# RaphaelHaddad/Real-Time-Brain-Inspired-Video-Memory

Hardware: NVIDIA B200
Metric: queries_per_sec_top10_384d (higher is better)
Workload: dtype tf32

## Files before the change

real-time-brain-inspired-video-memory_b200/csrc/api.cu:

```cuda
#include "common.cuh"

#include <dlfcn.h>
#include <stdarg.h>
#include <stdlib.h>
#include <string.h>
#include <time.h>
#include <new>
#include <vector>

namespace vm {

static thread_local char g_err[512] = "";
void set_error(const char *fmt, ...)
{
    va_list ap;
    va_start(ap, fmt);
    vsnprintf(g_err, sizeof(g_err), fmt, ap);
    va_end(ap);
}

int k_convert_rows(const void *src, int src_dtype, void *dst, int dst_dtype, int64_t n, int dim, int ld, cudaStream_t st);
int k_row_inv_norms(const void *rows, int dtype, float *inv_norms, int64_t row0, int64_t n, int ld, int *extreme, cudaStream_t st,
                    const double *exact = nullptr);
int k_invalidate_rows(float *inv_norms, const int64_t *rows_dev, int64_t n, int64_t size, cudaStream_t st);
// ... 217 lines not shown
static int ws_prepare(vm_store *s)
{
    Workspace &w = s->ws;
    if (w.ready) return VM_OK;
    int lists = 2 * s->sm_count;
    w.lists_max = lists;
    int rc;
#define ENS(b, bytes) if ((rc = (b).ensure(bytes)) != VM_OK) return rc
    ENS(w.q_raw, (size_t)MAXQ * s->dim * 8);
    ENS(w.q_f32, (size_t)MAXQ * s->ld * 4);
    ENS(w.q_bf16, (size_t)2 * MAXQ * s->ld * 2);
    ENS(w.cand, (size_t)lists * MAXQ * (MAXK > SCAN_SLAB ? MAXK : SCAN_SLAB) * 8);
    ENS(w.merged, (size_t)MAXQ * MAXK * 8);
    ENS(w.o_idx, result_bytes(MAXQ, MAXK) + 64);
    ENS(w.flags, (size_t)(MAXQ + 2) * 4);
    ENS(w.seed, (size_t)(SEED_TAB_WORDS + 3 * MAXQ) * 4);
    ENS(w.ubuf, (size_t)MAXQ * SCAN_UNION_CAP * 8);
    ENS(w.done, 64);
    ENS(w.scnt, (size_t)256 * MAXQ * 4);
    ENS(w.sel_inc, (size_t)MAXQ * 4);
    VM_CUDA_CHECK(cudaMemset(w.done.p, 0, 64));
    ENS(w.col_thr, (size_t)MAXQ * 4);
    ENS(w.col_cnt, (size_t)MAXQ * 4);
    ENS(w.col_buf, (size_t)MAXQ * COLLECT_CAP * 8);
    ENS(w.xs, (size_t)XCTAS * MAXQ * MAXK * 8);
    ENS(w.xr, (size_t)XCTAS * MAXQ * MAXK * 4);
    ENS(w.xc, (size_t)XCTAS * MAXQ * 4);
    ENS(w.taken, (size_t)MAXQ * XCTAS * MAXK);
#undef ENS
    VM_CUDA_CHECK(cudaMallocHost((void **)&w.h_uncert, 64));
    VM_CUDA_CHECK(cudaMallocHost((void **)&w.h_pack, result_bytes(MAXQ, MAXK) + 64));
// ... 973 lines not shown
    }
    delete c;
    return VM_OK;
}
extern "C" int vm_comm_nranks(const vm_comm *c) { return c ? c->nranks : -1; }
extern "C" int vm_comm_rank(const vm_comm *c) { return c ? c->rank : -1; }

extern "C" int vm_synth_fill(int device, void *rows_dev, int dtype, uint64_t seed, int64_t row0, int64_t n, int dim,
                             uint64_t dup_period, void *stream)
{
    VM_REQUIRE(rows_dev, VM_ERR_BADARG, "rows is NULL");
    VM_REQUIRE(dtype == VM_F32 || dtype == VM_BF16, VM_ERR_BADARG, "dtype must be VM_F32 or VM_BF16");
    DeviceGuard g(device);
    return k_synth_fill(rows_dev, dtype, seed, row0, n, dim, ld_for_dim(dim), dup_period, (cudaStream_t)stream);
}
```

real-time-brain-inspired-video-memory_b200/csrc/common.cuh:

```cuda
#pragma once
#include <cuda_runtime.h>
#include <cuda_bf16.h>
#include <stdint.h>
#include <stdio.h>
#include <math.h>
#include <utility>
#include "../../include/vidmem.h"

namespace vm {

void set_error(const char *fmt, ...);
#define VM_CUDA_CHECK(expr)                                                                      \
    do {                                                                                         \
        cudaError_t _e = (expr);                                                                 \
        if (_e != cudaSuccess) {                                                                 \
            vm::set_error("%s failed: %s (%s:%d)", #expr, cudaGetErrorString(_e), __FILE__, __LINE__); \
            return VM_ERR_CUDA;                                                                  \
        }                                                                                        \
    } while (0)
#define VM_REQUIRE(cond, code, ...)          \
    do {                                     \
        if (!(cond)) {                       \
            vm::set_error(__VA_ARGS__);      \
            return (code);                   \
// ... 16 lines not shown
    cfg.numAttrs = pdl ? 1 : 0;
    return cudaLaunchKernelEx(&cfg, kernel, std::forward<Args>(args)...);
}

template <auto Kernel>
static inline cudaError_t max_smem_once(int bytes)
{
    static bool set[64] = {};
    int dev = 0;
    cudaError_t e = cudaGetDevice(&dev);
    if (e != cudaSuccess || set[dev & 63]) return e;
    e = cudaFuncSetAttribute(Kernel, cudaFuncAttributeMaxDynamicSharedMemorySize, bytes);
    if (e == cudaSuccess) set[dev & 63] = true;
    return e;
}

__host__ __device__ __forceinline__ uint32_t f32_ordered(float f)
{
#ifdef __CUDA_ARCH__
    uint32_t b = __float_as_uint(f);
#else
    uint32_t b;
    memcpy(&b, &f, 4);
#endif
    return (b & 0x80000000u) ? ~b : (b | 0x80000000u);
}
__host__ __device__ __forceinline__ float f32_from_ordered(uint32_t o)
{
    uint32_t b = (o & 0x80000000u) ? (o & 0x7FFFFFFFu) : ~o;
#ifdef __CUDA_ARCH__
// ... 222 lines not shown
```

real-time-brain-inspired-video-memory_b200/csrc/scan_tc.cu:

```cuda
#include "tc_common.cuh"

namespace vm {
using namespace tc;

static constexpr int TC_BLOCK_M = 128;
static constexpr int TC_STAGE_BYTES = TC_BLOCK_M * 128;
static constexpr int TC_ACC = 8;
static constexpr int TC_THREADS_SVC = 288;
static constexpr int TC_THREADS = 192;
static constexpr int TC_TMEM_COLS = 512;
static constexpr int TC_MAX_STAGES = 8;

struct CollectArgs {
    const float *thr;
    uint64_t *buf;
    int *cnt;
    int cap;
    const int *pending;
};

struct BandArgs {
    uint64_t *slab;
    int *scnt;
    uint64_t *ubuf;
    int *ucnt;
    int ucap;
    float band;
    int ksel;
    int use_seed;
};

struct TcLayout {
    int nq_pad, KB, stages, split;
    uint32_t off_b, off_a, off_tauf, off_lcnt, off_cmax, off_wmax, off_flags, off_bars, off_tmem, total;
};

static TcLayout make_layout(int dtype, int ld, int nq, int split = 0)
{
    TcLayout L{};
    const int es = dtype == VM_F32 ? 4 : 2;
    L.nq_pad = (nq + 15) & ~15;
    L.KB = (ld * es + 127) / 128;
    L.split = (split && dtype == VM_BF16) ? 1 : 0;
    uint32_t o = 0;
    L.off_b = o; o += (uint32_t)L.KB * L.nq_pad * 128 * (L.split ? 2 : 1);
    const uint32_t epi = (uint32_t)L.nq_pad * (4 + 4 + 4 + 16) + 64 + 8 * (2 * TC_MAX_STAGES + 1 + 2 * TC_ACC) + 16;
    int64_t room = 227 * 1024 - 2048 - (int64_t)o - epi;
    L.stages = (int)(room / TC_STAGE_BYTES);
    if (L.stages > TC_MAX_STAGES) L.stages = TC_MAX_STAGES;
    if (L.stages < 0) L.stages = 0;
    L.off_a = o; o += (uint32_t)L.stages * TC_STAGE_BYTES;
    L.off_tauf = o; o += (uint32_t)L.nq_pad * 4;
    L.off_lcnt = o; o += (uint32_t)L.nq_pad * 4;
    L.off_cmax = o; o += (uint32_t)L.nq_pad * 4;
    L.off_wmax = o; o += (uint32_t)L.nq_pad * 16;
    L.off_flags = o; o += 64;
    L.off_bars = o; o += 8 * (2 * TC_MAX_STAGES + 1 + 2 * TC_ACC);
    L.off_tmem = o; o += 16;
    L.total = o + 1024;
#ifdef VIDMEM_AB_SMEMPAD
    if (L.total < 220 * 1024) L.total = 220 * 1024;
#endif
    return L;
}

__device__ __forceinline__ uint32_t own_kth_score(const uint64_t *slab, int n, int k, int lane)
{
    constexpr int PER = SCAN_SLAB / 32;
    uint32_t vals[PER];
#pragma unroll
    for (int t = 0; t < PER; ++t) {
        const int i = lane + 32 * t;
        vals[t] = i < n ? (uint32_t)(__ldcg(slab + i) >> 32) : 0u;
// ... 3 lines not shown
    for (int bit = 31; bit >= 12; --bit) {
        const uint32_t hi = bit == 31 ? 0u : (0xFFFFFFFFu << (bit + 1));
        int cnt = 0;
#pragma unroll
        for (int t = 0; t < PER; ++t) cnt += ((vals[t] & hi) == prefix && ((vals[t] >> bit) & 1u)) ? 1 : 0;
        const int tot = __reduce_add_sync(0xffffffffu, cnt);
        if (tot >= need) prefix |= 1u << bit;
        else need -= tot;
    }
    int ge = 0;
#pragma unroll
    for (int t = 0; t < PER; ++t) ge += (vals[t] != 0u && vals[t] >= prefix) ? 1 : 0;
    ge = __reduce_add_sync(0xffffffffu, ge);
    return (ge >= k && prefix != 0u) ? prefix : 0u;
}

template <bool TF32, bool DUMP, bool SPLIT>
__global__ void __launch_bounds__(DUMP ? TC_THREADS : TC_THREADS_SVC, 1)
scan_tc_kernel(const __grid_constant__ CUtensorMap tmA, const __grid_constant__ CUtensorMap tmB,
               const float *__restrict__ inv_norms, int64_t n, int num_tiles, int nq, TcLayout L, uint64_t *__restrict__ dump_keys,
               uint32_t *__restrict__ seed_tab, int *__restrict__ seed_ctr, CollectArgs col, BandArgs ub, int svc_sleep)
{
    const bool collect = !DUMP && col.thr != nullptr;
#ifndef VIDMEM_AB_NOPDL
    pdl_launch_dependents();
#endif
    if (collect) {
        pdl_wait();
        if (*col.pending == 0) return;
    }

    extern __shared__ __align__(16) uint8_t smem_raw[];
    uint8_t *base = smem_raw + ((1024u - (smem_u32(smem_raw) & 1023u)) & 1023u);
    uint8_t *sB = base + L.off_b;
    uint8_t *sA = base + L.off_a;
    float *tauf = (float *)(base + L.off_tauf);
    int *lcnt = (int *)(base + L.off_lcnt);
    uint32_t *cmax = (uint32_t *)(base + L.off_cmax);
    uint32_t *wmax = (uint32_t *)(base + L.off_wmax);
    volatile int *s_done = (volatile int *)(base + L.off_flags);
    uint64_t *bars = (uint64_t *)(base + L.off_bars);
    uint64_t *full = bars, *empty = bars + TC_MAX_STAGES, *qfull = bars + 2 * TC_MAX_STAGES;
    uint64_t *tfull = qfull + 1, *tempty = tfull + TC_ACC;
    uint32_t *tmem_slot = (uint32_t *)(base + L.off_tmem);

    const int warp = __shfl_sync(0xffffffffu, threadIdx.x >> 5, 0);
    const int lane = threadIdx.x & 31;
    const int nq_pad = L.nq_pad, KB = L.KB, stages = L.stages;
    constexpr int ELEMS = TF32 ? 32 : 64;

    if (warp == 0 && lane == 0) {
        tma_prefetch_desc(&tmA);
        tma_prefetch_desc(&tmB);
        for (int s = 0; s < stages; ++s) { mbar_init(&full[s], 1); mbar_init(&empty[s], 1); }
        mbar_init(qfull, 1);
        for (int a = 0; a < TC_ACC; ++a) { mbar_init(&tfull[a], 1); mbar_init(&tempty[a], 4); }
        fence_barrier_init();
    }
    if (warp == 1) tmem_alloc(tmem_slot, TC_TMEM_COLS);
#ifndef VIDMEM_AB_NOPDL
    if (!collect) pdl_wait();
#endif
    if (warp >= 2 && warp < 6) {
        const int e = threadIdx.x - 64;
        if (e < nq_pad) {
            lcnt[e] = 0;
            cmax[e] = 0u;
            tauf[e] = collect ? (e < nq ? col.thr[e] : INFINITY) : (e < nq ? -INFINITY : INFINITY);
        }
        if (e < 2) s_done[e] = 0;
    }
    tc_fence_before();
    __syncthreads();
    tc_fence_after();
    const uint32_t tmem_base = *tmem_slot;
    uint32_t *gbound = seed_tab ? seed_tab + SEED_TAB_WORDS : nullptr;

    if (warp == 0) {
        if (elect_one()) {
            constexpr int QPARTS = SPLIT ? 2 : 1;
            mbar_arrive_expect_tx(qfull, (uint32_t)(KB * QPARTS) * nq_pad * 128);
            for (int part = 0; part < QPARTS; ++part)
                for (int kb = 0; kb < KB; ++kb)
                    tma_load_2d(&tmB, qfull, sB + (size_t)(part * KB + kb) * nq_pad * 128, kb * ELEMS, part * nq_pad, L2_EVICT_LAST);
        }
        __syncwarp();
        int stage = 0;
        uint32_t phase = 0;
        for (int tile = blockIdx.x; tile < num_tiles; tile += gridDim.x) {
            for (int kb = 0; kb < KB; ++kb) {
                mbar_wait(&empty[stage], phase ^ 1);
                if (elect_one()) {
                    mbar_arrive_expect_tx(&full[stage], TC_STAGE_BYTES);
                    tma_load_2d(&tmA, &full[stage], sA + (size_t)stage * TC_STAGE_BYTES, kb * ELEMS, tile * TC_BLOCK_M, L2_EVICT_FIRST);
                }
                __syncwarp();
                if (++stage == stages) { stage = 0; phase ^= 1; }
            }
        }
    } else if (warp == 1) {
        const uint32_t idesc = make_idesc(TF32 ? 2u : 1u, TC_BLOCK_M, (uint32_t)nq_pad);
        mbar_wait(qfull, 0);
        tc_fence_after();
        int stage = 0, acc = 0;
        uint32_t phase = 0, acc_phase = 0;
        const uint64_t da0 = make_smem_desc_sw128(smem_u32(sA)), db0 = make_smem_desc_sw128(smem_u32(sB));
        const uint32_t kb_step = (uint32_t)(nq_pad * 128) >> 4, lo_step = (uint32_t)(KB * nq_pad * 128) >> 4;
        for (int tile = blockIdx.x; tile < num_tiles; tile += gridDim.x) {
            mbar_wait(&tempty[acc], acc_phase ^ 1);
            tc_fence_after();
            const uint32_t d_tmem = tmem_base + (uint32_t)(acc * nq_pad);
            for (int kb = 0; kb < KB; ++kb) {
                mbar_wait(&full[stage], phase);
                tc_fence_after();
                if (elect_one()) {
                    const uint64_t da = da0 + (uint64_t)((uint32_t)stage * (TC_STAGE_BYTES >> 4));
                    const uint64_t db = db0 + (uint64_t)((uint32_t)kb * kb_step);
#pragma unroll
                    for (int j = 0; j < 4; ++j) {
                        umma<TF32>(d_tmem, da + 2 * j, db + 2 * j, idesc, (uint32_t)((kb | j) != 0));
                        if constexpr (SPLIT) umma<TF32>(d_tmem, da + 2 * j, db + lo_step + 2 * j, idesc, 1u);
                    }
                    umma_commit(&empty[stage]);
                    if (kb == KB - 1) umma_commit(&tfull[acc]);
                }
                __syncwarp();
                if (++stage == stages) { stage = 0; phase ^= 1; }
            }
            if (++acc == TC_ACC) { acc = 0; acc_phase ^= 1; }
        }
    } else if (warp < 6) {
        const int e = threadIdx.x - 64;
        const int quad = warp & 3;
        const int row_in_tile = quad * 32 + lane;
        int acc = 0;
        uint32_t acc_phase = 0;
        if constexpr (DUMP) {
            for (int tile = blockIdx.x; tile < num_tiles; tile += gridDim.x) {
                const int64_t r = (int64_t)tile * TC_BLOCK_M + row_in_tile;
                const float iv = r < n ? __ldg(inv_norms + r) : -1.0f;
                mbar_wait(&tfull[acc], acc_phase);
                tc_fence_after();
                const uint32_t taddr = tmem_base + ((uint32_t)(quad * 32) << 16) + (uint32_t)(acc * nq_pad);
                uint64_t *out = dump_keys + (int64_t)tile * nq * TC_BLOCK_M + row_in_tile;
                for (int c = 0; c < nq_pad; c += 16) {
                    uint32_t v[16];
                    tmem_ld16(taddr + c, v);
                    tmem_ld_wait();
#pragma unroll
                    for (int j = 0; j < 16; ++j)
                        if (c + j < nq)
                            out[(int64_t)(c + j) * TC_BLOCK_M] = iv >= 0.0f ? make_key(__uint_as_float(v[j]) * iv, (uint32_t)r) : 0ull;
                }
                tc_fence_before();
                __syncwarp();
                if (lane == 0) mbar_arrive(&tempty[acc]);
                if (++acc == TC_ACC) { acc = 0; acc_phase ^= 1; }
            }
        } else {
        if (ub.use_seed && !collect) {
            const int64_t row0 = (int64_t)blockIdx.x * TC_BLOCK_M + row_in_tile;
            const float inv0 = row0 < n ? __ldg(inv_norms + row0) : -1.0f;
            mbar_wait(&tfull[0], 0);
            tc_fence_after();
            const uint32_t taddr0 = tmem_base + ((uint32_t)(quad * 32) << 16);
            for (int c = 0; c < nq_pad; c += 16) {
                uint32_t v[16];
                tmem_ld16(taddr0 + c, v);
                tmem_ld_wait();
#pragma unroll
                for (int j = 0; j < 16; ++j) {
                    const float sc = inv0 >= 0.0f ? __uint_as_float(v[j]) * inv0 : -INFINITY;
                    const uint32_t mx = __reduce_max_sync(0xffffffffu, f32_ordered(sc));
                    if (lane == 0) wmax[(warp - 2) * nq_pad + c + j] = mx;
                }
            }
            named_bar_sync(1, 128);
            if (e < nq_pad) {
// ... 28 lines not shown
                    const long long t0 = clock64();
                    while (*(volatile int *)pub_ctr < nq)
                        if (clock64() - t0 > 200000) break;
                    __threadfence();
                }
            }
            named_bar_sync(1, 128);
            if (e < nq) {
                const uint32_t o = __ldcg(gbound + e);
                if (o != 0u) tauf[e] = band_floor(f32_from_ordered(o), ub.band);
            }
            named_bar_sync(1, 128);
        }
        if (!collect && e == 0) s_done[1] = 1;
        uint64_t *my_slab = collect ? nullptr : ub.slab + (size_t)blockIdx.x * nq * SCAN_SLAB;
        int64_t row = (int64_t)blockIdx.x * TC_BLOCK_M + row_in_tile;
        float inv = row < n ? __ldg(inv_norms + row) : -1.0f;
        for (int tile = blockIdx.x; tile < num_tiles; tile += gridDim.x) {
            const int64_t row_next = row + (int64_t)gridDim.x * TC_BLOCK_M;
            const float inv_next = (tile + (int)gridDim.x < num_tiles && row_next < n) ? __ldg(inv_norms + row_next) : -1.0f;
            const bool valid = inv >= 0.0f;
            mbar_wait(&tfull[acc], acc_phase);
            tc_fence_after();
            const uint32_t taddr = tmem_base + ((uint32_t)(quad * 32) << 16) + (uint32_t)(acc * nq_pad);
            auto process = [&](const uint32_t (&v)[16], int c) {
                float tf[16];
#pragma unroll
                for (int j4 = 0; j4 < 4; ++j4) {
                    const float4 t4 = *reinterpret_cast<const float4 *>(tauf + c + 4 * j4);
                    tf[4 * j4] = t4.x; tf[4 * j4 + 1] = t4.y; tf[4 * j4 + 2] = t4.z; tf[4 * j4 + 3] = t4.w;
                }
                if (valid) {
                    uint32_t hits = 0;
#pragma unroll
                    for (int j = 0; j < 16; ++j) hits |= (__uint_as_float(v[j]) * inv >= tf[j]) ? (1u << j) : 0u;
// ... 41 lines not shown
                if (c + 16 < nq_pad) {
                    tmem_ld_wait();
                    if (c + 32 < nq_pad) tmem_ld16(taddr + c + 32, va);
                    process(vb, c + 16);
                }
            }
#ifdef VIDMEM_AB_TILEBAR
            named_bar_sync(1, 128);
#endif
            tc_fence_before();
            __syncwarp();
            if (lane == 0) mbar_arrive(&tempty[acc]);
            if (++acc == TC_ACC) { acc = 0; acc_phase ^= 1; }
            row = row_next;
            inv = inv_next;
        }
        if (!collect) {
            named_bar_sync(1, 128);
            if (e < nq) {
                ub.scnt[(size_t)blockIdx.x * nq + e] = lcnt[e];
                if (seed_tab != nullptr) __stcg(seed_tab + (size_t)blockIdx.x * nq_pad + e, cmax[e]);
            }
        }
        }
        __syncwarp();
        if (lane == 0) atomicAdd((int *)s_done, 1);
    } else {
#ifdef VIDMEM_AB_NOSVC
        if (false) {
#else
        if (!DUMP && warp == 8 && seed_tab != nullptr && !collect) {
#endif
            const int G = (int)gridDim.x;
// ... 59 lines not shown
                    if (q < nq) {
                        const uint32_t o = __ldcg(gbound + q);
                        if (o != 0u) {
                            const float f = band_floor(f32_from_ordered(o), ub.band);
                            if (f > tauf[q]) *(volatile float *)(tauf + q) = f;
                        }
                    }
                }
                __nanosleep(svc_sleep);
            }
        }
    }

    tc_fence_before();
    __syncthreads();
    if (warp == 1) {
        tc_fence_after();
        tmem_dealloc(tmem_base, TC_TMEM_COLS);
    }
}

bool scan_tc_supported(int dtype, int dim, int nq, int kp, int split)
{
    (void)kp;
    if (dtype != VM_F32 && dtype != VM_BF16) return false;
    if (nq < 1 || nq > 64) return false;
    TcLayout L = make_layout(dtype, ld_for_dim(dim), nq, split);
    return L.stages >= 3;
}

// ... 52 lines not shown
```

real-time-brain-inspired-video-memory_b200/csrc/select.cu:

```cuda
#include "common.cuh"

#include <type_traits>

namespace vm {

static constexpr int MERGE_THREADS = 512;
static constexpr int MERGE_SURV = 1024;

__device__ uint64_t radix_select_kth(const uint64_t *skeys, int total, int kp, int *hist, int *s_bin, int *s_need)
{
    const int tid = threadIdx.x, lane = tid & 31;
    uint64_t prefix = 0;
    int need = kp;
    for (int pass = 0; pass < 8; ++pass) {
        const int shift = 56 - 8 * pass;
        const uint64_t hmask = pass == 0 ? 0ull : (~0ull << (shift + 8));
        if (tid < 256) hist[tid] = 0;
        __syncthreads();
        for (int e = tid; e < total; e += MERGE_THREADS) {
            const uint64_t k = skeys[e];
            const bool act = k != 0 && (k & hmask) == prefix;
            const int bin = act ? (int)((k >> shift) & 0xFF) : -1;
            const unsigned peers = __match_any_sync(__activemask(), bin);
            if (act && (__ffs(peers) - 1) == lane) atomicAdd(&hist[bin], __popc(peers));
// ... 442 lines not shown
    int lists, list_len;
    int complete;
    const uint64_t *slab;
    const int *scnt;
    int ctas;
    const uint64_t *ubuf;
    const int *ucnt;
    int ucap;
    const uint32_t *seed_tab;
    int nq_pad, ksel;
    float band;
    int key_cap;
    int band_cap;
};

template <int THREADS>
__device__ int load_slab_keys(const SelectSrc &src, int q, int nq, uint64_t *skeys, int *s_cnts, int *s_total, float *s_bf, bool *incomplete)
{
    const int tid = threadIdx.x, lane = tid & 31, warp = tid >> 5;
    if (warp == 0) {
        float Lb = -INFINITY;
        if (src.seed_tab != nullptr) {
            if (src.ctas >= src.ksel) Lb = seed_select(src.seed_tab, src.ctas, src.nq_pad, q, src.ksel, lane);
            const uint32_t o = __ldcg(src.seed_tab + SEED_TAB_WORDS + q);
            if (o != 0u) Lb = fmaxf(Lb, f32_from_ordered(o));
        }
        if (lane == 0) { *s_bf = band_floor(Lb, src.band); *s_total = 0; }
    }
    for (int c = tid; c < src.ctas; c += THREADS) s_cnts[c] = min(src.scnt[(size_t)c * nq + q], SCAN_SLAB);
    __syncthreads();
    const float bf = *s_bf;
    constexpr int WARPS = THREADS / 32, PER = SCAN_SLAB / 32, BATCH = 4;
    for (int c0 = warp; c0 < src.ctas; c0 += WARPS * BATCH) {
        uint64_t kk[BATCH][PER];
#pragma unroll
        for (int b = 0; b < BATCH; ++b) {
            const int c = c0 + b * WARPS;
            const int cnt = c < src.ctas ? s_cnts[c] : 0;
#pragma unroll
            for (int t = 0; t < PER; ++t)
                kk[b][t] = (lane + 32 * t < cnt) ? __ldcg(src.slab + ((size_t)c * nq + q) * SCAN_SLAB + lane + 32 * t) : 0ull;
        }
#pragma unroll
        for (int b = 0; b < BATCH; ++b)
#pragma unroll
            for (int t = 0; t < PER; ++t) {
                const uint64_t k = kk[b][t];
                if (k != 0 && key_score(k) >= bf) {
                    const int p = atomicAdd(s_total, 1);
                    if (p < src.key_cap) skeys[p] = k;
                }
            }
    }
    const int spilled = src.ucnt[q];
    const int ns = min(spilled, src.ucap);
    for (int e = tid; e < ns; e += THREADS) {
        const uint64_t k = __ldcg(src.ubuf + (size_t)q * src.ucap + e);
        if (k != 0 && key_score(k) >= bf) {
            const int p = atomicAdd(s_total, 1);
            if (p < src.key_cap) skeys[p] = k;
        }
    }
    __syncthreads();
    const int got = *s_total;
    *incomplete = spilled > src.ucap || got > src.key_cap;
    return min(got, src.key_cap);
}

__global__ void __launch_bounds__(SR_THREADS) slab_top_kernel(SelectSrc src, int nq, int kp, uint64_t *__restrict__ merged,
                                                             int *__restrict__ incomplete)
{
    extern __shared__ __align__(16) unsigned char st_smem[];
    uint64_t *skeys = reinterpret_cast<uint64_t *>(st_smem);
    __shared__ int s_cnts[256];
    __shared__ int s_total, s_bin, s_need, s_m;
    __shared__ int hist[256];
    __shared__ float s_bf;
    const int q = blockIdx.x, tid = threadIdx.x;
    bool inc = false;
    const int total = load_slab_keys<SR_THREADS>(src, q, nq, skeys, s_cnts, &s_total, &s_bf, &inc);
    for (int e = tid; e < kp; e += SR_THREADS) merged[(int64_t)q * kp + e] = 0;
    if (tid == 0) { incomplete[q] = inc ? 1 : 0; s_m = 0; }
    __syncthreads();
    if (total <= MERGE_SURV) {
        for (int e = tid; e < total; e += SR_THREADS) {
            const uint64_t k = skeys[e];
            int rank = 0;
            for (int i = 0; i < total; ++i) rank += skeys[i] > k ? 1 : 0;
            if (rank < kp) merged[(int64_t)q * kp + rank] = k;
        }
        return;
    }
    const uint64_t Tk = radix_select_kth(skeys, total, kp, hist, &s_bin, &s_need);
    for (int e = tid; e < total; e += SR_THREADS) {
        const uint64_t k = skeys[e];
// ... 11 lines not shown
                                                                   const int *__restrict__ extreme, float *__restrict__ collect_thr,
                                                                   unsigned long long *__restrict__ cum, const float *__restrict__ inv_norms)
{
    extern __shared__ __align__(16) unsigned char sr_smem[];
    uint64_t *skeys = reinterpret_cast<uint64_t *>(sr_smem);
    uint32_t *lmax = reinterpret_cast<uint32_t *>(skeys + src.key_cap);
    double *sq = reinterpret_cast<double *>(lmax + ((src.lists + 3) & ~3));
    const int pitch = ld * (int)sizeof(T) + 16;
    unsigned char *srow = reinterpret_cast<unsigned char *>(sq + ((dim + 1) & ~1));
    double *b_sc = reinterpret_cast<double *>(srow + (((size_t)kp * pitch + 15) & ~(size_t)15));
    uint32_t *b_row = reinterpret_cast<uint32_t *>(b_sc + src.band_cap);
    __shared__ uint64_t s_top[64];
    __shared__ uint32_t s_rid[64];
    __shared__ uint64_t surv[MERGE_SURV];
    __shared__ int hist[256];
    __shared__ int s_bin, s_need, s_m, s_nz, s_cnt, s_band, s_viol, s_out, s_total;
    __shared__ int s_cnts[256];
    __shared__ uint32_t s_L;
    __shared__ float s_thr, s_bf;
    __shared__ double s_dot[64], s_rr[64], s_qq, s_score[64];
    const int q = blockIdx.x, tid = threadIdx.x, lane = tid & 31, warp = tid >> 5;

    pdl_launch_dependents();
    if (tid == 0) { s_m = 0; s_nz = 0; s_cnt = 0; s_band = 0; s_viol = 0; s_thr = -INFINITY; }
    if (tid < 64) s_top[tid] = 0;
    pdl_wait();
    __syncthreads();

    const bool union_mode = src.slab != nullptr;
    int total, lists = src.lists, list_len = src.list_len;
    bool overflow = false;
    int nz = 0;
    if (union_mode) {
        total = load_slab_keys<SR_THREADS>(src, q, nq, skeys, s_cnts, &s_total, &s_bf, &overflow);
        lists = 0;
        if (tid == 0) nz = total;
    } else {
        total = lists * list_len;
#pragma unroll 10
        for (int e = tid; e < total; e += SR_THREADS) {
            const int l = e / list_len, j = e - l * list_len;
            const uint64_t k = src.cand[((int64_t)l * nq + q) * list_len + j];
            skeys[e] = k;
            nz += k != 0;
        }
    }
    for (int i = tid; i < dim; i += SR_THREADS) sq[i] = load_as_double(queries, q_dtype, (int64_t)q * dim + i);
    if (nz) atomicAdd(&s_nz, nz);
    __syncthreads();
    const int nonzero = s_nz;
    bool done = false;
    if (total <= MERGE_SURV) {
        for (int e = tid; e < total; e += SR_THREADS) {
            const uint64_t k = skeys[e];
            if (k == 0) continue;
            int rank = 0;
            for (int i = 0; i < total; ++i) rank += skeys[i] > k ? 1 : 0;
            if (rank < kp) s_top[rank] = k;
        }
        done = true;
    } else if (nonzero >= kp && lists >= kp && lists <= 256) {
        for (int l = warp; l < lists; l += SR_THREADS / 32) {
            uint32_t m = 0;
            for (int j = lane; j < list_len; j += 32) m = max(m, (uint32_t)(skeys[l * list_len + j] >> 32));
// ... 44 lines not shown
    if (!done) {
        __syncthreads();
        uint64_t Tk = 1;
        if (nonzero >= kp) Tk = radix_select_kth(skeys, total, kp, hist, &s_bin, &s_need);
        if (tid == 0) s_m = 0;
        __syncthreads();
        for (int e = tid; e < total; e += SR_THREADS) {
            const uint64_t k = skeys[e];
            if (k >= Tk && k != 0) {
                if (nonzero >= kp && k == Tk) s_top[kp - 1] = k;
                else s_top[atomicAdd(&s_m, 1)] = k;
            }
        }
    }
    __syncthreads();

    const int j = tid;
    const uint64_t mykey = j < 64 ? s_top[j] : 0;
    const bool cand_valid = j < kp && mykey != 0;
    if (j < 64) s_rid[j] = cand_valid ? key_row(mykey) : NO_ROW;
    __syncthreads();
    stage_and_chain<NEUMAIER, T, SR_THREADS>(rows, ld, dim, kp, s_rid, srow, pitch, sq, s_dot, s_rr, &s_qq);

    double sc = 0.0;
    const uint32_t row = cand_valid ? key_row(mykey) : 0;
    const double n1 = __dsqrt_rn(s_qq);
    if (n1 == 0.0) {
        if (tid == 0) {
            int c = 0;
            const double outv = convert_score(0.0, f.score_mode);
            if (outv > f.min_score)
                for (int64_t r = 0; r < n_rows && c < f.k; ++r)
                    if (__ldg(inv_norms + r) >= 0.0f) {
                        f.out_idx[(int64_t)q * f.k + c] = r + f.row_offset;
                        f.out_score[(int64_t)q * f.k + c] = outv;
                        ++c;
                    }
// ... 230 lines not shown

static constexpr int XS_THREADS = 256;
static constexpr int XS_CG = 24;
static constexpr int XS_PITCH = XS_CG * 16 + 16;

template <bool NEUMAIER, typename T>
__global__ void __launch_bounds__(XS_THREADS) exact_scan_kernel(const T *__restrict__ rows, const float *__restrict__ inv_norms,
                                                               int64_t n, int ld, int dim, const void *__restrict__ queries,
                                                               int q_dtype, int nq, int32_t *__restrict__ flags, int k,
                                                               double *__restrict__ xlist_score, uint32_t *__restrict__ xlist_row,
                                                               int32_t *__restrict__ xlist_cnt, unsigned long long *__restrict__ cum,
                                                               int *__restrict__ done_ctr, FinalizeArgs f, uint8_t *__restrict__ taken)
{
    pdl_launch_dependents();
    pdl_wait();
    if (flags && flags[nq] == 0) return;
    if (flags && cum && blockIdx.x == 0 && threadIdx.x == 0) atomicAdd(cum + 3, (unsigned long long)flags[nq]);
    extern __shared__ __align__(16) unsigned char xs_smem[];
    double *sq = reinterpret_cast<double *>(xs_smem);
    unsigned char *buf0 = reinterpret_cast<unsigned char *>(sq + ((dim + 1) & ~1));
    __shared__ double l_score[XK], n_score[XK];
    __shared__ uint32_t l_row[XK], n_row[XK];
    __shared__ double c_score[128];
    __shared__ uint32_t c_row[128];
    __shared__ double s_dotv[128], s_rrv[128];
    __shared__ int l_cnt, c_cnt;
    __shared__ double s_n1;
    const int tid = threadIdx.x, rt = tid & 127;
    const bool is_rr = tid >= 128;
    const int gpr = ld * (int)sizeof(T) / 16;
// ... 495 lines not shown
```

real-time-brain-inspired-video-memory_b200/csrc/store.cu:

```cuda
#include "common.cuh"
#include "synth.cuh"

namespace vm {

template <typename DST>
__global__ void convert_rows_kernel(const void *__restrict__ src, int src_dtype, DST *__restrict__ dst, int64_t n,
                                    int dim, int ld)
{
    int64_t total = n * (int64_t)ld;
    for (int64_t e = blockIdx.x * (int64_t)blockDim.x + threadIdx.x; e < total; e += (int64_t)gridDim.x * blockDim.x) {
        int64_t r = e / ld;
        int c = (int)(e - r * ld);
        double dv = 0.0;
        if (c < dim) dv = load_as_double(src, src_dtype, r * dim + c);
        if constexpr (sizeof(DST) == 8) dst[e] = dv;
        else {
            const float v = (float)dv;
            if constexpr (sizeof(DST) == 4) dst[e] = v;
            else dst[e] = __float2bfloat16_rn(v);
        }
    }
}

template <typename T>
// ... 29 lines not shown
                if (extreme && (ss < 7.52316384526264e-37 || ss > 1.329227995784916e+36)) atomicAdd(extreme, 1);
            } else if (exact != nullptr && se != 0.0) {
                if (extreme) atomicAdd(extreme, 1);
            }
            inv_norms[r] = inv;
        }
    }
}

__global__ void invalidate_rows_kernel(float *inv_norms, const int64_t *rows, int64_t n, int64_t size)
{
    int64_t i = blockIdx.x * (int64_t)blockDim.x + threadIdx.x;
    if (i < n && rows[i] >= 0 && rows[i] < size) inv_norms[rows[i]] = -1.0f;
}

__global__ void normalize_queries_kernel(const void *__restrict__ q, int q_dtype, int nq, int nq_pad, int dim, int ld,
                                         float *__restrict__ out_f32, __nv_bfloat16 *__restrict__ out_bf16,
                                         int32_t *__restrict__ zero_me, uint32_t *__restrict__ zero_tab, int zero_tab_n,
                                         int tf32_round, int split)
{
    pdl_launch_dependents();
    pdl_wait();
    if (zero_me && blockIdx.x == 0 && threadIdx.x < 2) zero_me[threadIdx.x] = 0;
    for (int i = blockIdx.x * blockDim.x + threadIdx.x; i < zero_tab_n; i += gridDim.x * blockDim.x) zero_tab[i] = 0u;
    int lane = threadIdx.x & 31;
    int w = (blockIdx.x * blockDim.x + threadIdx.x) >> 5;
    if (w >= nq_pad) return;
    double ss = 0.0;
    if (w < nq)
        for (int c = lane; c < dim; c += 32) {
            double v = load_as_double(q, q_dtype, (int64_t)w * dim + c);
            ss += v * v;
        }
    for (int o = 16; o > 0; o >>= 1) ss += __shfl_xor_sync(0xffffffffu, ss, o);
    double inv = (ss > 0.0 && isfinite(ss)) ? 1.0 / sqrt(ss) : 0.0;
    for (int c = lane; c < ld; c += 32) {
        float v = 0.0f;
// ... 106 lines not shown
```

Baseline: 263,000.

## Dynamically schedule scan tiles via atomic counter and flatten slab-key loading

The tensor-core scan kernel now hands out tiles dynamically. The producer warp claims the next tile with a global atomic counter and passes tile ids to the MMA and epilogue warps through a shared-memory ring guarded by mbarriers, replacing static strided assignment. This is meant to even out load across CTAs. In select, slab keys are gathered with a block-wide prefix sum and a flat, unrolled load loop instead of per-warp batches. The first surviving candidate rows are prefetched into L2, and the query load is moved ahead of key loading to overlap it. Optional globaltimer stamps are added behind a compile flag. The changes add atomic and mbarrier overhead, and the tile counter only works if it is reset correctly between calls.

```diff
diff --git a/real-time-brain-inspired-video-memory_b200/csrc/api.cu b/real-time-brain-inspired-video-memory_b200/csrc/api.cu
--- a/real-time-brain-inspired-video-memory_b200/csrc/api.cu
+++ b/real-time-brain-inspired-video-memory_b200/csrc/api.cu
@@ -255,7 +255,7 @@
     ENS(w.merged, (size_t)MAXQ * MAXK * 8);
     ENS(w.o_idx, result_bytes(MAXQ, MAXK) + 64);
     ENS(w.flags, (size_t)(MAXQ + 2) * 4);
-    ENS(w.seed, (size_t)(SEED_TAB_WORDS + 3 * MAXQ) * 4);
+    ENS(w.seed, (size_t)(SEED_TAB_WORDS + 3 * MAXQ + 4) * 4);
     ENS(w.ubuf, (size_t)MAXQ * SCAN_UNION_CAP * 8);
     ENS(w.done, 64);
     ENS(w.scnt, (size_t)256 * MAXQ * 4);
@@ -1259,3 +1259,23 @@
     DeviceGuard g(device);
     return k_synth_fill(rows_dev, dtype, seed, row0, n, dim, ld_for_dim(dim), dup_period, (cudaStream_t)stream);
 }
+
+#ifdef VIDMEM_AB_STAMPS
+namespace vm {
+int ab_read_ab_norm(void *dst);
+int ab_read_ab_scan(void *dst);
+int ab_read_ab_sel(void *dst);
+int ab_read_ab_exact(void *dst);
+}
+extern "C" size_t vm_ab_stamps_bytes(void) { return sizeof(vm::AbRing); }
+extern "C" int vm_ab_stamps(int device, int which, void *dst)
+{
+    VM_REQUIRE(dst && which >= 0 && which < 4, VM_ERR_BADARG, "vm_ab_stamps: bad arguments");
+    DeviceGuard g(device);
+    VM_CUDA_CHECK(cudaDeviceSynchronize());
+    const int rc = which == 0 ? vm::ab_read_ab_norm(dst) : which == 1 ? vm::ab_read_ab_scan(dst) : which == 2 ? vm::ab_read_ab_sel(dst)
+                                                                                                 : vm::ab_read_ab_exact(dst);
+    VM_REQUIRE(rc == VM_OK, rc, "vm_ab_stamps: copy failed");
+    return VM_OK;
+}
+#endif
diff --git a/real-time-brain-inspired-video-memory_b200/csrc/common.cuh b/real-time-brain-inspired-video-memory_b200/csrc/common.cuh
--- a/real-time-brain-inspired-video-memory_b200/csrc/common.cuh
+++ b/real-time-brain-inspired-video-memory_b200/csrc/common.cuh
@@ -54,6 +54,37 @@
     if (e == cudaSuccess) set[dev & 63] = true;
     return e;
 }
+
+#ifdef VIDMEM_AB_STAMPS
+static constexpr int AB_RING = 128, AB_CTAS = 256, AB_FIELDS = 8;
+struct AbRing {
+    unsigned long long t[AB_RING][AB_CTAS][AB_FIELDS];
+    unsigned int tickets;
+};
+__device__ __forceinline__ unsigned long long ab_now()
+{
+    unsigned long long t;
+    asm volatile("mov.u64 %0, %%globaltimer;" : "=l"(t));
+    return t;
+}
+__device__ __forceinline__ int ab_ticket(AbRing *r) { return (int)((atomicAdd(&r->tickets, 1u) / gridDim.x) % AB_RING); }
+__device__ __forceinline__ void ab_put(AbRing *r, int slot, int field, unsigned long long t)
+{
+    if (blockIdx.x < AB_CTAS) r->t[slot][blockIdx.x][field] = t;
+}
+struct AbExitStamp {
+    AbRing *r;
+    int slot, field;
+    bool on;
+    __device__ ~AbExitStamp() { if (on) ab_put(r, slot, field, ab_now()); }
+};
+#define AB_STAMP(...) __VA_ARGS__
+#define AB_RING_DEFINE(NAME)                                                                                      \
+    static __device__ AbRing NAME;                                                                                \
+    int ab_read_##NAME(void *dst) { return cudaMemcpyFromSymbol(dst, NAME, sizeof(AbRing)) == cudaSuccess ? VM_OK : VM_ERR_CUDA; }
+#else
+#define AB_STAMP(...)
+#endif
 
 __host__ __device__ __forceinline__ uint32_t f32_ordered(float f)
 {
diff --git a/real-time-brain-inspired-video-memory_b200/csrc/scan_tc.cu b/real-time-brain-inspired-video-memory_b200/csrc/scan_tc.cu
--- a/real-time-brain-inspired-video-memory_b200/csrc/scan_tc.cu
+++ b/real-time-brain-inspired-video-memory_b200/csrc/scan_tc.cu
@@ -10,6 +10,7 @@
 static constexpr int TC_THREADS = 192;
 static constexpr int TC_TMEM_COLS = 512;
 static constexpr int TC_MAX_STAGES = 8;
+static constexpr int TC_TILE_RING = 16;
 
 struct CollectArgs {
     const float *thr;
@@ -32,7 +33,7 @@
 
 struct TcLayout {
     int nq_pad, KB, stages, split;
-    uint32_t off_b, off_a, off_tauf, off_lcnt, off_cmax, off_wmax, off_flags, off_bars, off_tmem, total;
+    uint32_t off_b, off_a, off_tauf, off_lcnt, off_cmax, off_wmax, off_flags, off_bars, off_tmem, off_ring, total;
 };
 
 static TcLayout make_layout(int dtype, int ld, int nq, int split = 0)
@@ -44,7 +45,7 @@
     L.split = (split && dtype == VM_BF16) ? 1 : 0;
     uint32_t o = 0;
     L.off_b = o; o += (uint32_t)L.KB * L.nq_pad * 128 * (L.split ? 2 : 1);
-    const uint32_t epi = (uint32_t)L.nq_pad * (4 + 4 + 4 + 16) + 64 + 8 * (2 * TC_MAX_STAGES + 1 + 2 * TC_ACC) + 16;
+    const uint32_t epi = (uint32_t)L.nq_pad * (4 + 4 + 4 + 16) + 64 + 8 * (2 * TC_MAX_STAGES + 1 + 2 * TC_ACC) + 16 + TC_TILE_RING * (4 + 16);
     int64_t room = 227 * 1024 - 2048 - (int64_t)o - epi;
     L.stages = (int)(room / TC_STAGE_BYTES);
     if (L.stages > TC_MAX_STAGES) L.stages = TC_MAX_STAGES;
@@ -57,6 +58,7 @@
     L.off_flags = o; o += 64;
     L.off_bars = o; o += 8 * (2 * TC_MAX_STAGES + 1 + 2 * TC_ACC);
     L.off_tmem = o; o += 16;
+    L.off_ring = o; o += TC_TILE_RING * (4 + 16);
     L.total = o + 1024;
 #ifdef VIDMEM_AB_SMEMPAD
     if (L.total < 220 * 1024) L.total = 220 * 1024;
@@ -90,6 +92,8 @@
     ge = __reduce_add_sync(0xffffffffu, ge);
     return (ge >= k && prefix != 0u) ? prefix : 0u;
 }
+
+AB_STAMP(AB_RING_DEFINE(ab_scan))
 
 template <bool TF32, bool DUMP, bool SPLIT>
 __global__ void __launch_bounds__(DUMP ? TC_THREADS : TC_THREADS_SVC, 1)
@@ -119,6 +123,9 @@
     uint64_t *full = bars, *empty = bars + TC_MAX_STAGES, *qfull = bars + 2 * TC_MAX_STAGES;
     uint64_t *tfull = qfull + 1, *tempty = tfull + TC_ACC;
     uint32_t *tmem_slot = (uint32_t *)(base + L.off_tmem);
+    int *tring = (int *)(base + L.off_ring);
+    uint64_t *tready = (uint64_t *)(base + L.off_ring + TC_TILE_RING * 4), *tfree = tready + TC_TILE_RING;
+    AB_STAMP(int &ab_slot_s = ((int *)(base + L.off_flags))[4];)
 
     const int warp = __shfl_sync(0xffffffffu, threadIdx.x >> 5, 0);
     const int lane = threadIdx.x & 31;
@@ -131,12 +138,14 @@
         for (int s = 0; s < stages; ++s) { mbar_init(&full[s], 1); mbar_init(&empty[s], 1); }
         mbar_init(qfull, 1);
         for (int a = 0; a < TC_ACC; ++a) { mbar_init(&tfull[a], 1); mbar_init(&tempty[a], 4); }
+        for (int r = 0; r < TC_TILE_RING; ++r) { mbar_init(&tready[r], 1); mbar_init(&tfree[r], 5); }
         fence_barrier_init();
     }
     if (warp == 1) tmem_alloc(tmem_slot, TC_TMEM_COLS);
 #ifndef VIDMEM_AB_NOPDL
     if (!collect) pdl_wait();
 #endif
+    AB_STAMP(if (threadIdx.x == 64) { ab_slot_s = ab_ticket(&ab_scan); ab_put(&ab_scan, ab_slot_s, 0, ab_now()); })
     if (warp >= 2 && warp < 6) {
         const int e = threadIdx.x - 64;
         if (e < nq_pad) {
@@ -151,6 +160,15 @@
     tc_fence_after();
     const uint32_t tmem_base = *tmem_slot;
     uint32_t *gbound = seed_tab ? seed_tab + SEED_TAB_WORDS : nullptr;
+    int *tile_ctr = (!DUMP && !collect && seed_tab) ? (int *)(seed_tab + SEED_TAB_WORDS + 3 * 64) : nullptr;
+    auto take_tile = [&](int j) -> int {
+        const int s = j % TC_TILE_RING;
+        mbar_wait(&tready[s], (uint32_t)(j / TC_TILE_RING) & 1u);
+        const int t = *(volatile int *)(tring + s);
+        __syncwarp();
+        if (lane == 0) mbar_arrive(&tfree[s]);
+        return t;
+    };
 
     if (warp == 0) {
         if (elect_one()) {
@@ -163,8 +181,17 @@
         __syncwarp();
         int stage = 0;
         uint32_t phase = 0;
-        for (int tile = blockIdx.x; tile < num_tiles; tile += gridDim.x) {
+        const int kb_claim = KB > stages ? KB - stages : 0;
+        int tile = (int)blockIdx.x < num_tiles ? (int)blockIdx.x : -1;
+        for (int j = 0;; ++j) {
+            const int s = j % TC_TILE_RING;
+            mbar_wait(&tfree[s], ((uint32_t)(j / TC_TILE_RING) & 1u) ^ 1u);
+            if (lane == 0) { tring[s] = tile; mbar_arrive(&tready[s]); }
+            __syncwarp();
+            if (tile < 0) break;
+            int claim = 0;
             for (int kb = 0; kb < KB; ++kb) {
+                if (tile_ctr && kb == kb_claim && lane == 0) claim = atomicAdd(tile_ctr, 1);
                 mbar_wait(&empty[stage], phase ^ 1);
                 if (elect_one()) {
                     mbar_arrive_expect_tx(&full[stage], TC_STAGE_BYTES);
@@ -173,6 +200,8 @@
                 __syncwarp();
                 if (++stage == stages) { stage = 0; phase ^= 1; }
             }
+            const int next = tile_ctr ? (int)gridDim.x + __shfl_sync(0xffffffffu, claim, 0) : tile + (int)gridDim.x;
+            tile = next < num_tiles ? next : -1;
         }
     } else if (warp == 1) {
         const uint32_t idesc = make_idesc(TF32 ? 2u : 1u, TC_BLOCK_M, (uint32_t)nq_pad);
@@ -182,12 +211,13 @@
         uint32_t phase = 0, acc_phase = 0;
         const uint64_t da0 = make_smem_desc_sw128(smem_u32(sA)), db0 = make_smem_desc_sw128(smem_u32(sB));
         const uint32_t kb_step = (uint32_t)(nq_pad * 128) >> 4, lo_step = (uint32_t)(KB * nq_pad * 128) >> 4;
-        for (int tile = blockIdx.x; tile < num_tiles; tile += gridDim.x) {
+        for (int j = 0; take_tile(j) >= 0; ++j) {
             mbar_wait(&tempty[acc], acc_phase ^ 1);
             tc_fence_after();
             const uint32_t d_tmem = tmem_base + (uint32_t)(acc * nq_pad);
             for (int kb = 0; kb < KB; ++kb) {
                 mbar_wait(&full[stage], phase);
+                AB_STAMP(if (j == 0 && kb == 0 && lane == 0) ab_put(&ab_scan, ab_slot_s, 1, ab_now());)
                 tc_fence_after();
                 if (elect_one()) {
                     const uint64_t da = da0 + (uint64_t)((uint32_t)stage * (TC_STAGE_BYTES >> 4));
@@ -212,7 +242,9 @@
         int acc = 0;
         uint32_t acc_phase = 0;
         if constexpr (DUMP) {
-            for (int tile = blockIdx.x; tile < num_tiles; tile += gridDim.x) {
+            for (int j = 0;; ++j) {
+                const int tile = take_tile(j);
+                if (tile < 0) break;
                 const int64_t r = (int64_t)tile * TC_BLOCK_M + row_in_tile;
                 const float iv = r < n ? __ldg(inv_norms + r) : -1.0f;
                 mbar_wait(&tfull[acc], acc_phase);
@@ -238,6 +270,7 @@
             const int64_t row0 = (int64_t)blockIdx.x * TC_BLOCK_M + row_in_tile;
             const float inv0 = row0 < n ? __ldg(inv_norms + row0) : -1.0f;
             mbar_wait(&tfull[0], 0);
+            AB_STAMP(if (e == 0) ab_put(&ab_scan, ab_slot_s, 2, ab_now());)
             tc_fence_after();
             const uint32_t taddr0 = tmem_base + ((uint32_t)(quad * 32) << 16);
             for (int c = 0; c < nq_pad; c += 16) {
@@ -296,11 +329,14 @@
         }
         if (!collect && e == 0) s_done[1] = 1;
         uint64_t *my_slab = collect ? nullptr : ub.slab + (size_t)blockIdx.x * nq * SCAN_SLAB;
-        int64_t row = (int64_t)blockIdx.x * TC_BLOCK_M + row_in_tile;
-        float inv = row < n ? __ldg(inv_norms + row) : -1.0f;
-        for (int tile = blockIdx.x; tile < num_tiles; tile += gridDim.x) {
-            const int64_t row_next = row + (int64_t)gridDim.x * TC_BLOCK_M;
-            const float inv_next = (tile + (int)gridDim.x < num_tiles && row_next < n) ? __ldg(inv_norms + row_next) : -1.0f;
+        int j = 0;
+        int tile = take_tile(j++);
+        int64_t row = (int64_t)tile * TC_BLOCK_M + row_in_tile;
+        float inv = (tile >= 0 && row < n) ? __ldg(inv_norms + row) : -1.0f;
+        while (tile >= 0) {
+            const int tile_next = take_tile(j++);
+            const int64_t row_next = (int64_t)tile_next * TC_BLOCK_M + row_in_tile;
+            const float inv_next = (tile_next >= 0 && row_next < n) ? __ldg(inv_norms + row_next) : -1.0f;
             const bool valid = inv >= 0.0f;
             mbar_wait(&tfull[acc], acc_phase);
             tc_fence_after();
@@ -372,9 +408,11 @@
             if (++acc == TC_ACC) { acc = 0; acc_phase ^= 1; }
             row = row_next;
             inv = inv_next;
+            tile = tile_next;
         }
         if (!collect) {
             named_bar_sync(1, 128);
+            AB_STAMP(if (e == 0) ab_put(&ab_scan, ab_slot_s, 3, ab_now());)
             if (e < nq) {
                 ub.scnt[(size_t)blockIdx.x * nq + e] = lcnt[e];
                 if (seed_tab != nullptr) __stcg(seed_tab + (size_t)blockIdx.x * nq_pad + e, cmax[e]);
@@ -464,6 +502,7 @@
 
     tc_fence_before();
     __syncthreads();
+    AB_STAMP(if (threadIdx.x == 0) ab_put(&ab_scan, ab_slot_s, 4, ab_now());)
     if (warp == 1) {
         tc_fence_after();
         tmem_dealloc(tmem_base, TC_TMEM_COLS);
diff --git a/real-time-brain-inspired-video-memory_b200/csrc/select.cu b/real-time-brain-inspired-video-memory_b200/csrc/select.cu
--- a/real-time-brain-inspired-video-memory_b200/csrc/select.cu
+++ b/real-time-brain-inspired-video-memory_b200/csrc/select.cu
@@ -3,6 +3,9 @@
 #include <type_traits>
 
 namespace vm {
+
+AB_STAMP(AB_RING_DEFINE(ab_sel))
+AB_STAMP(AB_RING_DEFINE(ab_exact))
 
 static constexpr int MERGE_THREADS = 512;
 static constexpr int MERGE_SURV = 1024;
@@ -480,55 +483,104 @@
     int band_cap;
 };
 
+static constexpr int SELECT_PREFETCH_ROWS = 64;
 template <int THREADS>
-__device__ int load_slab_keys(const SelectSrc &src, int q, int nq, uint64_t *skeys, int *s_cnts, int *s_total, float *s_bf, bool *incomplete)
-{
+__device__ int load_slab_keys(const SelectSrc &src, int q, int nq, uint64_t *skeys, int *s_off, int *s_aux, float *s_bf, bool *incomplete,
+                              const char *pf_rows = nullptr, int pf_row_bytes = 0)
+{
+    static_assert(THREADS >= 256, "one thread per slab count");
     const int tid = threadIdx.x, lane = tid & 31, warp = tid >> 5;
+    const int cnt = tid < src.ctas ? min(src.scnt[(size_t)tid * nq + q], SCAN_SLAB) : 0;
+    if (tid == 256) s_aux[2] = src.ucnt[q];
     if (warp == 0) {
         float Lb = -INFINITY;
         if (src.seed_tab != nullptr) {
+            const uint32_t o = __ldcg(src.seed_tab + SEED_TAB_WORDS + q);
             if (src.ctas >= src.ksel) Lb = seed_select(src.seed_tab, src.ctas, src.nq_pad, q, src.ksel, lane);
-            const uint32_t o = __ldcg(src.seed_tab + SEED_TAB_WORDS + q);
             if (o != 0u) Lb = fmaxf(Lb, f32_from_ordered(o));
         }
-        if (lane == 0) { *s_bf = band_floor(Lb, src.band); *s_total = 0; }
-    }
-    for (int c = tid; c < src.ctas; c += THREADS) s_cnts[c] = min(src.scnt[(size_t)c * nq + q], SCAN_SLAB);
-    __syncthreads();
+        if (lane == 0) { *s_bf = band_floor(Lb, src.band); s_aux[0] = 0; }
+    }
+    int inc = cnt;
+#pragma unroll
+    for (int o = 1; o < 32; o <<= 1) {
+        const int v = __shfl_up_sync(0xffffffffu, inc, o);
+        if (lane >= o) inc += v;
+    }
+    if (warp < 8 && lane == 31) s_aux[8 + warp] = inc;
+    __syncthreads();
+    int before = 0, nslab = 0;
+#pragma unroll
+    for (int w = 0; w < 8; ++w) {
+        const int s = s_aux[8 + w];
+        before += w < warp ? s : 0;
+        nslab += s;
+    }
+    if (tid < 256) s_off[tid] = before + inc - cnt;
     const float bf = *s_bf;
-    constexpr int WARPS = THREADS / 32, PER = SCAN_SLAB / 32, BATCH = 4;
-    for (int c0 = warp; c0 < src.ctas; c0 += WARPS * BATCH) {
-        uint64_t kk[BATCH][PER];
-#pragma unroll
-        for (int b = 0; b < BATCH; ++b) {
-            const int c = c0 + b * WARPS;
-            const int cnt = c < src.ctas ? s_cnts[c] : 0;
-#pragma unroll
-            for (int t = 0; t < PER; ++t)
-                kk[b][t] = (lane + 32 * t < cnt) ? __ldcg(src.slab + ((size_t)c * nq + q) * SCAN_SLAB + lane + 32 * t) : 0ull;
-        }
-#pragma unroll
-        for (int b = 0; b < BATCH; ++b)
-#pragma unroll
-            for (int t = 0; t < PER; ++t) {
-                const uint64_t k = kk[b][t];
-                if (k != 0 && key_score(k) >= bf) {
-                    const int p = atomicAdd(s_total, 1);
-                    if (p < src.key_cap) skeys[p] = k;
+    const int spilled = s_aux[2];
+    const int ns = min(spilled, src.ucap);
+    __syncthreads();
+    const bool big = nslab > 4 * THREADS;
+    if (big) {
+        constexpr int WARPS = THREADS / 32, PER = SCAN_SLAB / 32, BATCH = 4;
+        for (int c0 = warp; c0 < src.ctas; c0 += WARPS * BATCH) {
+            uint64_t kk[BATCH][PER];
+#pragma unroll
+            for (int b = 0; b < BATCH; ++b) {
+                const int c = c0 + b * WARPS;
+                const int cn = c < src.ctas ? (c + 1 < src.ctas ? s_off[c + 1] : nslab) - s_off[c] : 0;
+#pragma unroll
+                for (int t = 0; t < PER; ++t)
+                    kk[b][t] = (lane + 32 * t < cn) ? __ldcg(src.slab + ((size_t)c * nq + q) * SCAN_SLAB + lane + 32 * t) : 0ull;
+            }
+#pragma unroll
+            for (int b = 0; b < BATCH; ++b)
+#pragma unroll
+                for (int t = 0; t < PER; ++t) {
+                    const uint64_t k = kk[b][t];
+                    if (k != 0 && key_score(k) >= bf) {
+                        const int p = atomicAdd(&s_aux[0], 1);
+                        if (p < src.key_cap) skeys[p] = k;
+                    }
                 }
-            }
-    }
-    const int spilled = src.ucnt[q];
-    const int ns = min(spilled, src.ucap);
-    for (int e = tid; e < ns; e += THREADS) {
-        const uint64_t k = __ldcg(src.ubuf + (size_t)q * src.ucap + e);
-        if (k != 0 && key_score(k) >= bf) {
-            const int p = atomicAdd(s_total, 1);
-            if (p < src.key_cap) skeys[p] = k;
-        }
-    }
-    __syncthreads();
-    const int got = *s_total;
+        }
+    }
+    const int total_in = nslab + ns;
+    constexpr int U = 4;
+    for (int i0 = tid + (big ? nslab : 0); i0 < total_in; i0 += U * THREADS) {
+        uint64_t kk[U];
+#pragma unroll
+        for (int u = 0; u < U; ++u) {
+            const int i = i0 + u * THREADS;
+            kk[u] = 0ull;
+            if (i < nslab) {
+                int lo = 0, hi = src.ctas - 1;
+                while (lo < hi) {
+                    const int mid = (lo + hi + 1) >> 1;
+                    if (s_off[mid] <= i) lo = mid;
+                    else hi = mid - 1;
+                }
+                kk[u] = __ldcg(src.slab + ((size_t)lo * nq + q) * SCAN_SLAB + (i - s_off[lo]));
+            } else if (i < total_in) {
+                kk[u] = __ldcg(src.ubuf + (size_t)q * src.ucap + (i - nslab));
+            }
+        }
+#pragma unroll
+        for (int u = 0; u < U; ++u) {
+            const uint64_t k = kk[u];
+            if (k != 0 && key_score(k) >= bf) {
+                const int p = atomicAdd(&s_aux[0], 1);
+                if (p < src.key_cap) skeys[p] = k;
+                if (pf_rows != nullptr && p < SELECT_PREFETCH_ROWS) {
+                    const char *r = pf_rows + (size_t)key_row(k) * pf_row_bytes;
+                    for (int l = 0; l < pf_row_bytes; l += 128) asm volatile("prefetch.global.L2 [%0];" ::"l"(r + l));
+                }
+            }
+        }
+    }
+    __syncthreads();
+    const int got = s_aux[0];
     *incomplete = spilled > src.ucap || got > src.key_cap;
     return min(got, src.key_cap);
 }
@@ -538,13 +590,13 @@
 {
     extern __shared__ __align__(16) unsigned char st_smem[];
     uint64_t *skeys = reinterpret_cast<uint64_t *>(st_smem);
-    __shared__ int s_cnts[256];
-    __shared__ int s_total, s_bin, s_need, s_m;
+    __shared__ int s_off[256], s_aux[16];
+    __shared__ int s_bin, s_need, s_m;
     __shared__ int hist[256];
     __shared__ float s_bf;
     const int q = blockIdx.x, tid = threadIdx.x;
     bool inc = false;
-    const int total = load_slab_keys<SR_THREADS>(src, q, nq, skeys, s_cnts, &s_total, &s_bf, &inc);
+    const int total = load_slab_keys<SR_THREADS>(src, q, nq, skeys, s_off, s_aux, &s_bf, &inc);
     for (int e = tid; e < kp; e += SR_THREADS) merged[(int64_t)q * kp + e] = 0;
     if (tid == 0) { incomplete[q] = inc ? 1 : 0; s_m = 0; }
     __syncthreads();
@@ -586,17 +638,21 @@
     __shared__ uint32_t s_rid[64];
     __shared__ uint64_t surv[MERGE_SURV];
     __shared__ int hist[256];
-    __shared__ int s_bin, s_need, s_m, s_nz, s_cnt, s_band, s_viol, s_out, s_total;
-    __shared__ int s_cnts[256];
+    __shared__ int s_bin, s_need, s_m, s_nz, s_cnt, s_band, s_viol, s_out;
+    __shared__ int s_off[256], s_aux[16];
     __shared__ uint32_t s_L;
     __shared__ float s_thr, s_bf;
     __shared__ double s_dot[64], s_rr[64], s_qq, s_score[64];
     const int q = blockIdx.x, tid = threadIdx.x, lane = tid & 31, warp = tid >> 5;
 
+    AB_STAMP(const unsigned long long ab_t0 = ab_now();)
     pdl_launch_dependents();
     if (tid == 0) { s_m = 0; s_nz = 0; s_cnt = 0; s_band = 0; s_viol = 0; s_thr = -INFINITY; }
     if (tid < 64) s_top[tid] = 0;
     pdl_wait();
+    for (int i = tid; i < dim; i += SR_THREADS) sq[i] = load_as_double(queries, q_dtype, (int64_t)q * dim + i);
+    AB_STAMP(int ab_slot = 0; if (tid == 0) { ab_slot = ab_ticket(&ab_sel); ab_put(&ab_sel, ab_slot, 0, ab_t0); ab_put(&ab_sel, ab_slot, 1, ab_now()); })
+    AB_STAMP(AbExitStamp ab_exit{&ab_sel, ab_slot, 5, tid == 0};)
     __syncthreads();
 
     const bool union_mode = src.slab != nullptr;
@@ -604,7 +660,8 @@
     bool overflow = false;
     int nz = 0;
     if (union_mode) {
-        total = load_slab_keys<SR_THREADS>(src, q, nq, skeys, s_cnts, &s_total, &s_bf, &overflow);
+        total = load_slab_keys<SR_THREADS>(src, q, nq, skeys, s_off, s_aux, &s_bf, &overflow, reinterpret_cast<const char *>(rows),
+                                           ld * (int)sizeof(T));
         lists = 0;
         if (tid == 0) nz = total;
     } else {
@@ -617,9 +674,9 @@
             nz += k != 0;
         }
     }
-    for (int i = tid; i < dim; i += SR_THREADS) sq[i] = load_as_double(queries, q_dtype, (int64_t)q * dim + i);
     if (nz) atomicAdd(&s_nz, nz);
     __syncthreads();
+    AB_STAMP(if (tid == 0) ab_put(&ab_sel, ab_slot, 2, ab_now());)
     const int nonzero = s_nz;
     bool done = false;
     if (total <= MERGE_SURV) {
@@ -694,6 +751,7 @@
         }
     }
     __syncthreads();
+    AB_STAMP(if (tid == 0) ab_put(&ab_sel, ab_slot, 3, ab_now());)
 
     const int j = tid;
     const uint64_t mykey = j < 64 ? s_top[j] : 0;
@@ -701,6 +759,7 @@
     if (j < 64) s_rid[j] = cand_valid ? key_row(mykey) : NO_ROW;
     __syncthreads();
     stage_and_chain<NEUMAIER, T, SR_THREADS>(rows, ld, dim, kp, s_rid, srow, pitch, sq, s_dot, s_rr, &s_qq);
+    AB_STAMP(if (tid == 0) ab_put(&ab_sel, ab_slot, 4, ab_now());)
 
     double sc = 0.0;
     const uint32_t row = cand_valid ? key_row(mykey) : 0;
@@ -961,6 +1020,8 @@
 {
     pdl_launch_dependents();
     pdl_wait();
+    AB_STAMP(int ab_slot = 0; if (threadIdx.x == 0) ab_slot = ab_ticket(&ab_exact);)
+    AB_STAMP(AbExitStamp ab_exit{&ab_exact, ab_slot, 0, threadIdx.x == 0};)
     if (flags && flags[nq] == 0) return;
     if (flags && cum && blockIdx.x == 0 && threadIdx.x == 0) atomicAdd(cum + 3, (unsigned long long)flags[nq]);
     extern __shared__ __align__(16) unsigned char xs_smem[];
diff --git a/real-time-brain-inspired-video-memory_b200/csrc/store.cu b/real-time-brain-inspired-video-memory_b200/csrc/store.cu
--- a/real-time-brain-inspired-video-memory_b200/csrc/store.cu
+++ b/real-time-brain-inspired-video-memory_b200/csrc/store.cu
@@ -67,6 +67,8 @@
     if (i < n && rows[i] >= 0 && rows[i] < size) inv_norms[rows[i]] = -1.0f;
 }
 
+AB_STAMP(AB_RING_DEFINE(ab_norm))
+
 __global__ void normalize_queries_kernel(const void *__restrict__ q, int q_dtype, int nq, int nq_pad, int dim, int ld,
                                          float *__restrict__ out_f32, __nv_bfloat16 *__restrict__ out_bf16,
                                          int32_t *__restrict__ zero_me, uint32_t *__restrict__ zero_tab, int zero_tab_n,
@@ -74,6 +76,8 @@
 {
     pdl_launch_dependents();
     pdl_wait();
+    AB_STAMP(int ab_slot = 0; if (threadIdx.x == 0) { ab_slot = ab_ticket(&ab_norm); ab_put(&ab_norm, ab_slot, 0, ab_now()); })
+    AB_STAMP(AbExitStamp ab_exit{&ab_norm, ab_slot, 1, threadIdx.x == 0};)
     if (zero_me && blockIdx.x == 0 && threadIdx.x < 2) zero_me[threadIdx.x] = 0;
     for (int i = blockIdx.x * blockDim.x + threadIdx.x; i < zero_tab_n; i += gridDim.x * blockDim.x) zero_tab[i] = 0u;
     int lane = threadIdx.x & 31;
```

Result: faster. 269,000 (median of 6 runs) (+2.3%).
